# HakimNessah/th_rl

Hardware: AMD Instinct MI355X
Metric: env-steps/sec, 2-agent PD x 1M parallel games (higher is better)
Workload: dtype f32

## Files before the change

### th_rl_amd/csrc/thrl_wave_kernel.h

```cpp
#pragma once
#include <type_traits>
#include <utility>
#include "thrl_kernels.h"
#include "thrl_wave_lut.h"

#ifndef THRL_ABLATE
#define THRL_ABLATE 0
#endif

namespace thrl {

constexpr int kAblate = THRL_ABLATE;

typedef unsigned int v2u __attribute__((ext_vector_type(2)));

__device__ __forceinline__ v2u pack_halves(unsigned a, unsigned b) {
    return __builtin_amdgcn_permlane32_swap(a, b, false, false);
}

__device__ __forceinline__ unsigned lds_addr(const void* p) {
    return (unsigned)(uintptr_t)(__attribute__((address_space(3))) const void*)p;
}
template <typename QT>
__device__ __forceinline__ QT lds_load(unsigned addr) {
    typedef __attribute__((address_space(3))) QT lds_t;
    return *(const lds_t*)(uintptr_t)addr;
}
template <typename QT>
__device__ __forceinline__ void lds_store(unsigned addr, QT v) {
    typedef __attribute__((address_space(3))) QT lds_t;
    *(lds_t*)(uintptr_t)addr = v;
}

__device__ __forceinline__ void lds_inc(unsigned addr) {
    typedef unsigned __attribute__((may_alias)) u32_alias;
    typedef __attribute__((address_space(3))) u32_alias lds_u32;
    __hip_atomic_fetch_add((lds_u32*)(uintptr_t)addr, 1u, __ATOMIC_RELAXED, __HIP_MEMORY_SCOPE_WAVEFRONT);
}
__device__ __forceinline__ void lds_zero8(unsigned addr) {
    typedef unsigned long long __attribute__((may_alias)) u64_alias;
    typedef __attribute__((address_space(3))) u64_alias lds_u64;
    *(lds_u64*)(uintptr_t)addr = 0ull;
}

__device__ __forceinline__ unsigned bperm(unsigned byte_sel, unsigned v) {
    return (unsigned)__builtin_amdgcn_ds_bpermute((int)byte_sel, (int)v);
}

template <int CTRL>
__device__ __forceinline__ double dpp_mov64(double v) {
    const int lo = __double2loint(v), hi = __double2hiint(v);
    return __hiloint2double(__builtin_amdgcn_update_dpp(hi, hi, CTRL, 0xF, 0xF, false),
                            __builtin_amdgcn_update_dpp(lo, lo, CTRL, 0xF, 0xF, false));
}
template <int CTRL>
__device__ __forceinline__ uint32_t dpp_mov32(uint32_t v) {
    return (uint32_t)__builtin_amdgcn_update_dpp((int)v, (int)v, CTRL, 0xF, 0xF, false);
}

__device__ __forceinline__ float group8_allmax(float v) {
    asm("s_nop 1\n\t"
        "v_max_f32_dpp %0, %0, %0 quad_perm:[1,0,3,2] row_mask:0xf bank_mask:0xf\n\t"
        "s_nop 1\n\t"
        "v_max_f32_dpp %0, %0, %0 quad_perm:[2,3,0,1] row_mask:0xf bank_mask:0xf\n\t"
        "s_nop 1\n\t"
        "v_max_f32_dpp %0, %0, %0 row_half_mirror row_mask:0xf bank_mask:0xf"
        : "+v"(v));
    return v;
}
__device__ __forceinline__ double group8_allmax(double v) {
    v = fmax(v, dpp_mov64<0xB1>(v));
    v = fmax(v, dpp_mov64<0x4E>(v));
    v = fmax(v, dpp_mov64<0x141>(v));
    return v;
}
__device__ __forceinline__ void store_where(unsigned long long mask, unsigned addr, float v) {
    unsigned long long save;
    asm volatile("s_mov_b64 %0, exec\n\ts_mov_b64 exec, %1\n\tds_write_b32 %2, %3\n\ts_mov_b64 exec, %0"
                 : "=&s"(save) : "s"(mask), "v"(addr), "v"(v) : "memory");
}
__device__ __forceinline__ void store_where(unsigned long long mask, unsigned addr, double v) {
    unsigned long long save;
    asm volatile("s_mov_b64 %0, exec\n\ts_mov_b64 exec, %1\n\tds_write_b64 %2, %3\n\ts_mov_b64 exec, %0"
                 : "=&s"(save) : "s"(mask), "v"(addr), "v"(v) : "memory");
}
__device__ __forceinline__ void store_lanes(unsigned long long mask, long long* base, unsigned off, double v) {
    asm volatile("s_mov_b64 exec, %0\n\tglobal_store_dwordx2 %1, %2, %3\n\ts_mov_b64 exec, -1"
                 :: "s"(mask), "v"(off), "v"(v), "s"(base) : "memory");
}
template <int IMM>
__device__ __forceinline__ void store_key(unsigned key, unsigned want, unsigned addr, float v) {
    if constexpr (IMM >= 0)
        asm volatile("v_cmpx_eq_u32 vcc, %0, %1\n\tds_write_b32 %2, %3\n\ts_mov_b64 exec, -1"
                     :: "n"(IMM), "v"(key), "v"(addr), "v"(v) : "memory", "vcc");
    else
        asm volatile("v_cmpx_eq_u32 vcc, %0, %1\n\tds_write_b32 %2, %3\n\ts_mov_b64 exec, -1"
                     :: "s"(want), "v"(key), "v"(addr), "v"(v) : "memory", "vcc");
}
template <int IMM>
__device__ __forceinline__ void store_key(unsigned key, unsigned want, unsigned addr, double v) {
    if constexpr (IMM >= 0)
        asm volatile("v_cmpx_eq_u32 vcc, %0, %1\n\tds_write_b64 %2, %3\n\ts_mov_b64 exec, -1"
                     :: "n"(IMM), "v"(key), "v"(addr), "v"(v) : "memory", "vcc");
    else
        asm volatile("v_cmpx_eq_u32 vcc, %0, %1\n\tds_write_b64 %2, %3\n\ts_mov_b64 exec, -1"
                     :: "s"(want), "v"(key), "v"(addr), "v"(v) : "memory", "vcc");
}
constexpr unsigned kKeyShift = 25;
constexpr unsigned kKeyNone = 0x7Fu;
__device__ __forceinline__ float dpp_ror8(float v) { return __builtin_bit_cast(float, dpp_mov32<0x128>(__builtin_bit_cast(uint32_t, v))); }
__device__ __forceinline__ double dpp_ror8(double v) { return dpp_mov64<0x128>(v); }
__device__ __forceinline__ float max_of(float a, float b) { return fmaxf(a, b); }
__device__ __forceinline__ double max_of(double a, double b);
__device__ __forceinline__ float half32_allmax(float v) {
    v = group8_allmax(v);
    v = fmaxf(v, __builtin_bit_cast(float, dpp_mov32<0x140>(__builtin_bit_cast(uint32_t, v))));
    unsigned a = __builtin_bit_cast(unsigned, v), b = a;
    asm("" : "+v"(b));
    const v2u r = __builtin_amdgcn_permlane16_swap(a, b, false, false);
    const unsigned rx = r.x, ry = r.y;
// ... 380 lines not shown
template <int L>
__device__ __forceinline__ uint32_t writelane_imm(uint32_t old, uint32_t val) {
    asm("v_writelane_b32 %0, %1, %2" : "+v"(old) : "s"(val), "n"(L));
    return old;
}
template <int T0>
__device__ __forceinline__ void chain_group_affine(uint32_t& sq, uint32_t& sc, uint32_t Tq) {
    const uint32_t s1 = readlane_u(Tq, (int)sc) & 0xFFu;
    const uint32_t s2 = (readlane_u(Tq, (int)s1) >> 8) & 0xFFu;
    const uint32_t s3 = (readlane_u(Tq, (int)s2) >> 16) & 0xFFu;
    const uint32_t s4 = readlane_u(Tq, (int)s3) >> 24;
    const uint32_t w = pack16(sc, s2) | (pack16(s1, s3) << 8);
    sq = writelane_imm<T0>(sq, w);
    sc = s4;
}
__device__ __forceinline__ uint32_t play_affine(int seg, int n, int lane, uint32_t rw, uint32_t G0q, uint32_t G1q, unsigned mk_addr,
                                                int c, int m0, int m1, int& s) {
    const int s_entry = __builtin_amdgcn_readfirstlane(s);
    {
        const uint32_t kb = (uint32_t)c - ((rw & 1u) ? ((rw >> 8) & 0xFFu) * (uint32_t)m0 : 0u)
                                        - ((rw & 2u) ? ((rw >> 16) & 0xFFu) * (uint32_t)m1 : 0u);
        const unsigned ad = mk_addr + 16u * (unsigned)(lane >> 2) + (unsigned)(lane & 3);
        lds_store<unsigned char>(ad, (rw & 1u) ? (unsigned char)0 : (unsigned char)0xFF);
        lds_store<unsigned char>(ad + 4u, (rw & 2u) ? (unsigned char)0 : (unsigned char)0xFF);
        lds_store<unsigned char>(ad + 8u, (unsigned char)kb);
        __builtin_amdgcn_wave_barrier();
    }
    struct Q4 { v2u lo, hi; };
    auto loadq = [&](int g) {
        Q4 q;
        q.lo = lds_load<v2u>(mk_addr + 16u * (unsigned)g);
        q.hi = lds_load<v2u>(mk_addr + 16u * (unsigned)g + 8u);
        return q;
    };
    auto make = [&](const Q4& q) {
        asm volatile("" :: "v"(q.hi.y));
        return q.hi.x - (G0q & q.lo.x) - (G1q & q.lo.y);
    };
    uint32_t sq = 0u, sq_tail = 0u;
    uint32_t sc = (uint32_t)s_entry & 0xFFu;
    auto chain4 = [&](auto t0c, const int nn, const uint32_t Tq) {
        constexpr int t0 = decltype(t0c)::value;
        __builtin_amdgcn_sched_barrier(0);
        if (t0 + 4 <= nn) chain_group_affine<t0>(sq, sc, Tq);
        else {
#pragma unroll
            for (int j = 0; j < 4; j++) {
                if (t0 + j < nn) {
                    sq_tail = writelane_u(sq_tail, sc * 0x101u, t0 + j);
                    sc = (readlane_u(Tq, (int)sc) >> (8 * j)) & 0xFFu;
                }
            }
        }
        __builtin_amdgcn_sched_barrier(0);
    };
    Q4 qa = loadq(0), qb = loadq(1);
    uint32_t Ta = make(qa), Tb = 0u;
#define THRL_PLAYA2(G, N_)                                                                   \
    if ((G) * 4 < (N_)) {                                                                    \
        if ((G) * 4 + 8 < (N_)) qa = loadq((G) + 2 < 15 ? (G) + 2 : 15);                     \
        chain4(std::integral_constant<int, (G) * 4>(), (N_), Ta);                            \
        if ((G) * 4 + 4 < (N_)) {                                                            \
            Tb = make(qb);                                                                   \
            if ((G) * 4 + 12 < (N_)) qb = loadq((G) + 3 < 15 ? (G) + 3 : 15);                \
            chain4(std::integral_constant<int, (G) * 4 + 4>(), (N_), Tb);                    \
            if ((G) * 4 + 8 < (N_)) Ta = make(qa);                                           \
        }                                                                                    \
    }
#define THRL_PLAYA16(N_)                                                                     \
    THRL_PLAYA2(0, N_) THRL_PLAYA2(2, N_) THRL_PLAYA2(4, N_) THRL_PLAYA2(6, N_)              \
    THRL_PLAYA2(8, N_) THRL_PLAYA2(10, N_) THRL_PLAYA2(12, N_) THRL_PLAYA2(14, N_)
    if (n == 64) { THRL_PLAYA16(64) } else if (n == 36) { THRL_PLAYA16(36) } else { THRL_PLAYA16(n) }
#undef THRL_PLAYA16
#undef THRL_PLAYA2
    s = (int)(sc * 0x101u);
    uint32_t qd;
    asm("s_nop 1\n\tv_mov_b32_dpp %0, %1 quad_perm:[0,0,0,0] row_mask:0xf bank_mask:0xf" : "=v"(qd) : "v"(sq));
    const uint32_t un = ((qd >> (8u * (unsigned)(lane & 3))) & 0xFFu) * 0x101u;
    uint32_t out = lane < (n & ~3) ? un : sq_tail;
    if (seg == 0) out = writelane_imm<0>(out, (uint32_t)s_entry);
    return out;
}

template <typename QT, int NSEG, int NRSEG, bool NOISE, bool SWEEP, bool CYCLE, bool GREEDY = false, bool LOG = false, bool AFFINE = false>
__global__ void __launch_bounds__(1024)
__attribute__((amdgpu_waves_per_eu(sizeof(QT) == 8 ? 3 : (NOISE ? 4 : (NSEG <= 2 ? 5 : 4)))))
k_wave_episodes(const WaveArgs a) {
    extern __shared__ __attribute__((aligned(16))) unsigned char smem[];
    static_assert(!AFFINE || (sizeof(QT) == 4 && !NOISE && !SWEEP && !CYCLE && !GREEDY && NRSEG == 1 && kAblate == 0),
                  "closed-form play tables: plain float32 variants with one row register");
    constexpr bool kUnrollReplay = NSEG <= 2 && !(NOISE && sizeof(QT) == 8);
    const int lane = threadIdx.x & 63;
    const int wib = __builtin_amdgcn_readfirstlane((int)(threadIdx.x >> 6));
    const int A = a.A, W = a.win_rows, Tenv = a.T, epk = CYCLE ? a.epk : 1, T = a.T * epk, lo = a.row_lo;
    const int replay_from = CYCLE ? a.replay_from : 0;
    const WaveLut L = wave_lut_layout(A);

    {
        const uint32_t* src = reinterpret_cast<const uint32_t*>(a.lut_ns);
        uint32_t* dst = reinterpret_cast<uint32_t*>(smem);
        for (int k = threadIdx.x; k < (a.lut_bytes >> 2); k += blockDim.x) dst[k] = src[k];
    }
    __syncthreads();
    const unsigned lut_ns_lds = lds_addr(smem + L.ns_off);
    const double* lut_aq = reinterpret_cast<const double*>(smem + L.aq_off);
    const double* lut_sct = reinterpret_cast<const double*>(smem + L.sct_off);

    QT* tab0 = reinterpret_cast<QT*>(smem + a.lut_bytes + (size_t)wib * a.game_lds_bytes);
    QT* tab1 = tab0 + (W + 2) * A;
    const int half = lane >> 5;
    const unsigned tab0_off = lds_addr(tab0);
    const unsigned tab1_off = lds_addr(tab1);
    const int kk = (lane >> 3) & 3, jj = lane & 7;
    const unsigned perm_sel = (unsigned)((lane & 32) + 4 * jj + kk) << 2;
    const unsigned my_step = (unsigned)(4 * jj + kk);
    const unsigned row_shift = (unsigned)(7 * kk);
    const unsigned row_bytes = (unsigned)A * (unsigned)sizeof(QT);
    const int rdn = A < 3 ? 2 : (A <= 24 ? 3 : 4);
    const unsigned rd_base = (half ? tab1_off : tab0_off) + (unsigned)sizeof(QT) * (unsigned)min(rdn * jj, A - rdn);
    constexpr bool kLdsMK = sizeof(QT) == 4 && !NOISE && !GREEDY && NRSEG == 1 && !(kAblate & 6);
    const unsigned mk_addr = tab0_off + 2u * (unsigned)((W + 2) * A) * (unsigned)sizeof(QT);
    constexpr bool kArgmax21 = sizeof(QT) == 4;
    constexpr bool kMaskSched = !NOISE && !GREEDY;
    constexpr bool kParkLogs = !LOG && !CYCLE;

    const AgentParams& p0 = a.ag[0];
    const AgentParams& p1 = a.ag[1];
    const double inv_T_den = (double)Tenv;

    long long acc = 0, acc_hi = 0;
    const double log_scale = (lane & 2) ? a.log_scale[1] : a.log_scale[0];
    const int wave_gid = blockIdx.x * a.waves_per_block + wib;
    auto load_parked = [&](int pass) {
        return __hip_atomic_load(&a.partial[(size_t)wave_gid * 128 + 64 * pass + lane], __ATOMIC_RELAXED, __HIP_MEMORY_SCOPE_AGENT);
    };
    auto finish_parked = [&](long long p0w, long long p1w) {
#pragma unroll
        for (int pass = 0; pass < 2; pass++) {
            if (pass == 1 && a.n_episodes <= 16) break;
            double v = __longlong_as_double(pass ? p1w : p0w);
            if ((lane & 3) < 2) v = __ddiv_rn(v, inv_T_den);
            const long long vq = __double2ll_rn(__dmul_rn(v, log_scale));
            if (16 * pass + (lane >> 2) < a.n_episodes) { if (pass) acc_hi += vq; else acc += vq; }
        }
    };

    int g_claim = 0;
    if (lane == 0) g_claim = atomicAdd(a.next_game, 1);
    for (;;) {
        const int g = __builtin_amdgcn_readfirstlane(g_claim);
        if (g >= a.G) break;
        if (lane == 0) g_claim = atomicAdd(a.next_game, 1);
        const uint64_t gid = a.game_offset + (uint64_t)g;
        QT* __restrict__ q0 = reinterpret_cast<QT*>(a.q) + (int64_t)g * a.stride + p0.table_off;
        QT* __restrict__ q1 = reinterpret_cast<QT*>(a.q) + (int64_t)g * a.stride + p1.table_off;
        const double price0 = a.state[g];

        QT gamma_h = half ? HP<QT>::gamma(p1) : HP<QT>::gamma(p0);
        QT alpha_h = half ? HP<QT>::alpha(p1) : HP<QT>::alpha(p0);
        QT oma0 = HP<QT>::one_minus_alpha(p0), oma1 = HP<QT>::one_minus_alpha(p1);
        if (SWEEP && a.sw_gamma) gamma_h = HP<QT>::from_double(a.sw_gamma[(size_t)half * a.G + g]);
        if (SWEEP && a.sw_alpha) {
            alpha_h = HP<QT>::from_double(a.sw_alpha[(size_t)half * a.G + g]);
            oma0 = HP<QT>::from_double(__dsub_rn(1.0, a.sw_alpha[g]));
            oma1 = HP<QT>::from_double(__dsub_rn(1.0, a.sw_alpha[(size_t)a.G + g]));
        }
        double epsg0 = 0.0, epsg1 = 0.0;
        const bool sw_eps_on = SWEEP && a.sw_eps != nullptr;
        if (sw_eps_on) { epsg0 = a.sw_eps[g]; epsg1 = a.sw_eps[(size_t)a.G + g]; }
        const QT ag_h = HP<QT>::product(alpha_h, gamma_h);
        const double eend0 = (SWEEP && a.sw_eps_end) ? a.sw_eps_end[g] : p0.eps_end;
        const double eend1 = (SWEEP && a.sw_eps_end) ? a.sw_eps_end[(size_t)a.G + g] : p1.eps_end;
        const double estep0 = (SWEEP && a.sw_eps_step) ? a.sw_eps_step[g] : p0.eps_step;
        const double estep1 = (SWEEP && a.sw_eps_step) ? a.sw_eps_step[(size_t)a.G + g] : p1.eps_step;
        const double noise_prob_g = (SWEEP && a.sw_noise_prob) ? a.sw_noise_prob[g] : a.env.noise_prob;

        {
            const QT* s0 = q0 + lo * A;
            const QT* s1 = q1 + lo * A;
            const int n = W * A;
            for (int k0 = 0; k0 < n; k0 += 512) {
                QT v0[8], v1[8];
#pragma unroll
                for (int j = 0; j < 8; j++) {
                    const int k = min(k0 + j * 64 + lane, n - 1);
                    v0[j] = s0[k]; v1[j] = s1[k];
                }
#pragma unroll
                for (int j = 0; j < 8; j++) {
                    const int k = k0 + j * 64 + lane;
                    if (k < n) { tab0[k] = v0[j]; tab1[k] = v1[j]; }
                }
            }
        }
        int sp = __builtin_amdgcn_readfirstlane(encode32(price0, p0));
        int st = __builtin_amdgcn_readfirstlane(encode64(price0, p0));
        sp = min(max(sp, 0), a.rows - 1);
        st = min(max(st, 0), a.rows - 1);
        int spill0 = -1, spill1 = -1, sp_l, st_l;
        if (sp >= lo && sp < lo + W) sp_l = sp - lo; else { spill0 = sp; sp_l = W; }
        if (st == sp) st_l = sp_l;
        else if (st >= lo && st < lo + W) st_l = st - lo;
        else { spill1 = st; st_l = W + 1; }

        {
            if (spill0 >= 0 && lane < A) {
                tab0[W * A + lane] = q0[spill0 * A + lane];
                tab1[W * A + lane] = q1[spill0 * A + lane];
            }
            if (spill1 >= 0 && lane < A) {
                tab0[(W + 1) * A + lane] = q0[spill1 * A + lane];
                tab1[(W + 1) * A + lane] = q1[spill1 * A + lane];
            }
        }
        __builtin_amdgcn_wave_barrier();

        int s = sp_l | (st_l << 8);
        double last_price = price0;
        for (int e = 0; e < a.n_episodes; e += epk) {
            const uint32_t eg = (uint32_t)(a.first_episode + (uint64_t)e);

            uint32_t AM[NRSEG], R[NRSEG];
            uint32_t G0q = 0u, G1q = 0u;
#pragma unroll
            for (int k = 0; k < NRSEG; k++) {
                const int row = min(lane + 64 * k, W + 1);
                const QT* r0 = tab0 + row * A;
                const QT* r1 = tab1 + row * A;
                QT b0 = r0[0], b1 = r1[0];
                uint32_t i0 = 0, i1 = 0;
                if (kAblate & 16) {
                } else if (kArgmax21 && A == 21) {
                    i0 = argmax21_first(tab0_off + (unsigned)row * 84u);
                    i1 = argmax21_first(tab1_off + (unsigned)row * 84u);
                } else if (A == 21) {
#pragma unroll
                    for (int j = 1; j < 21; j++) {
                        const QT v0 = r0[j], v1 = r1[j];
                        if (v0 > b0) { b0 = v0; i0 = j; }
                        if (v1 > b1) { b1 = v1; i1 = j; }
                    }
                } else {
#pragma unroll 4
                    for (int j = 1; j < A; j++) {
                        const QT v0 = r0[j], v1 = r1[j];
                        if (v0 > b0) { b0 = v0; i0 = j; }
                        if (v1 > b1) { b1 = v1; i1 = j; }
                    }
                }
                if (kAblate & 16) { i0 = (uint32_t)(lane * 5) % (uint32_t)A; i1 = (uint32_t)(lane * 3) % (uint32_t)A; }
                AM[k] = i0 | (i1 << 8);
                R[k] = (i0 * (uint32_t)A * 2u) | (i1 << 17);
                if constexpr (AFFINE) {
                    G0q = i0 * ((uint32_t)a.aff_m0 * 0x01010101u);
                    G1q = i1 * ((uint32_t)a.aff_m1 * 0x01010101u);
                }
            }
            GreedyTables<GREEDY && NRSEG == 1> gt;
            gt.build(halves_sum(R[0]) + lut_ns_lds);

            uint32_t seq[NSEG], rwv[NSEG];
            unsigned explored_segs = 0u;
            double nav[NSEG];
#pragma unroll
            for (int seg = 0; seg < NSEG; seg++) {
                int n = min(64, T - seg * 64);
                asm volatile("" : "+s"(n));
                uint32_t rw;
                nav[seg] = 0.0;
                const int tcl = min(seg * 64 + lane, T - 1);
                const int ep = epk == 1 ? 0 : tcl / Tenv;
                const uint32_t st_in_ep = (uint32_t)(tcl - ep * Tenv);
                double eps0, eps1;
                if (sw_eps_on) { eps0 = epsg0; eps1 = epsg1; }
                else if (epk == 1) { eps0 = a.eps[e][0]; eps1 = a.eps[e][1]; }
                else { eps0 = a.eps[e + ep][0]; eps1 = a.eps[e + ep][1]; }
                if (a.inj_u) {
                    const int tt = tcl;
                    const size_t k = (((size_t)e * Tenv + tt) * 2) * (size_t)a.G + (size_t)g;
                    const uint32_t ex0 = a.inj_u[k] < eps0 ? 1u : 0u;
                    const uint32_t ex1 = a.inj_u[k + a.G] < eps1 ? 2u : 0u;
                    const uint32_t c0 = min((uint32_t)(uint8_t)a.inj_choice[k], (uint32_t)(A - 1));
                    const uint32_t c1 = min((uint32_t)(uint8_t)a.inj_choice[k + a.G], (uint32_t)(A - 1));
                    rw = ex0 | ex1 | (c0 << 8) | (c1 << 16);
                } else if (kAblate & 8) {
                    const uint32_t h = (uint32_t)(lane * 2654435761u) ^ eg;
                    rw = (h & 3u) | (((h >> 4) % (uint32_t)A) << 8) | (((h >> 12) % (uint32_t)A) << 16);
                } else {
                    uint32_t seed_lo = (uint32_t)a.seed, seed_hi = (uint32_t)(a.seed >> 32);
                    asm volatile("" : "+s"(seed_lo), "+s"(seed_hi));
                    const uint64_t seed_here = ((uint64_t)seed_hi << 32) | seed_lo;
                    const u32x4 x = draw_lanes(seed_here, gid, eg + (uint32_t)ep, st_in_ep, 0u);
                    const uint32_t ex0 = u01_32(x.x) < eps0 ? 1u : 0u;
                    const uint32_t ex1 = u01_32(x.z) < eps1 ? 2u : 0u;
                    rw = ex0 | ex1 | (__umulhi(x.y, (uint32_t)A) << 8) | (__umulhi(x.w, (uint32_t)A) << 16);
// ... 289 lines not shown
                    const uint32_t c1 = h1 & 1u;
                    const uint32_t c2 = ((h2 >> 1) & 1u) | ((c1 ^ 1u) & h2 & 1u);
                    const uint32_t c3 = ((h3 >> 2) & 1u) | ((c2 ^ 1u) & (((h3 >> 1) & 1u) | ((c1 ^ 1u) & h3 & 1u)));
                    bool quad_quiet = true;
                    if (NOISE) quad_quiet = ((__ballot((rwv[seg] & 4u) != 0u) >> (lane & 60)) & 0xFull) == 0ull;
                    const uint32_t same4 = ((quad_quiet && b0 == b1 && b1 == b2 && b2 == b3 && (b0 >> 24) == ((b0 >> 16) & 0xFFu)) ||
                                            (GREEDY && b0 == b2 && b1 == b3 && (b0 >> 24) == ((b1 >> 16) & 0xFFu) &&
                                             (b1 >> 24) == ((b0 >> 16) & 0xFFu) && (b0 >> 24) != (b1 >> 24))) ? 1u : 0u;
                    cutq = (c1 | (c2 << 1) | (c3 << 2)) & ((uint32_t)(pairs >> quad0) >> 1);
                    P = (b0 >> 24) | ((b1 >> 24) << 7) | ((b2 >> 24) << 14) | ((b3 >> 24) << 21) |
                        (cutq << 28) | (same4 << 31);
                    any_fixed = __ballot((P >> 31) != 0u) != 0ull;
                }

                const uint32_t pass_no = (uint32_t)__builtin_popcount(cutq & ((1u << ((uint32_t)lane & 3u)) - 1u));
                const uint32_t key_base = tab0_off + ((trains ? (quad0 & 28u) + pass_no : kKeyNone) << kKeyShift);
                const v2u woq = pack_halves(key_base + (cwv[seg] & 0xFFFFu) * kCellScale, key_base + (cwv[seg] >> 16) * kCellScale);

                bool seg_done = false;
                if (GREEDY && !(kAblate & 257) && !((explored_segs >> seg) & 1u)) {
                    const int nseg = min(64, T - seg * 64);
                    const uint32_t w = act[seg];
                    const uint32_t w1 = dpp_mov32<0x138>(w), w2 = dpp_mov32<0x138>(w1);
                    const uint32_t w3 = dpp_mov32<0x138>(w2), w4 = dpp_mov32<0x138>(w3);
                    const bool in_seg = lane < nseg;
                    const int period = __ballot(in_seg && lane >= 1 && w != w1) == 0ull ? 1
                                     : __ballot(in_seg && lane >= 2 && w != w2) == 0ull ? 2
                                     : __ballot(in_seg && lane >= 3 && w != w3) == 0ull ? 3
                                     : __ballot(in_seg && lane >= 4 && w != w4) == 0ull ? 4 : 0;
                    if (period > 0 && nseg >= period) {
                        uint32_t W[4];
#pragma unroll
                        for (int j = 0; j < 4; j++) W[j] = readlane_u(w, j);
                        bool ok = true;
#pragma unroll
                        for (int j = 0; j < 4; j++)
                            if (j < period) {
                                const uint32_t nxt_row = (W[(j + 1 < period) ? j + 1 : 0] >> 16) & 0xFFu;
                                ok = ok && (W[j] >> 24) == nxt_row;
#pragma unroll
                                for (int i = 0; i < j; i++) ok = ok && ((W[i] >> 16) & 0xFFu) != ((W[j] >> 16) & 0xFFu);
                            }
                        if (ok) {
                            seg_done = true;
                            const BlockOps<QT> ops0 = make_ops(snap[seg], 0, r0d, r1d, alpha_h);
                            const unsigned tabh = half ? tab1_off : tab0_off;
                            const unsigned wo_step = woq.x & ((1u << kKeyShift) - 1u);
                            if (period == 1) cyclic_segment<QT, 1>(ops0, wo_step, W, nseg, lane, tabh, A, row_bytes, ag_h, alpha_h, gamma_h);
                            else if (period == 2) cyclic_segment<QT, 2>(ops0, wo_step, W, nseg, lane, tabh, A, row_bytes, ag_h, alpha_h, gamma_h);
                            else if (period == 3) cyclic_segment<QT, 3>(ops0, wo_step, W, nseg, lane, tabh, A, row_bytes, ag_h, alpha_h, gamma_h);
                            else cyclic_segment<QT, 4>(ops0, wo_step, W, nseg, lane, tabh, A, row_bytes, ag_h, alpha_h, gamma_h);
                            __builtin_amdgcn_wave_barrier();
                        }
                    }
                }
#pragma unroll
                for (int k = 0; k < 2; k++) {
                    if (GREEDY && seg_done) break;
                    int nsub = __builtin_amdgcn_readfirstlane(min(32, T - seg * 64 - k * 32));
                    asm volatile("" : "+s"(nsub));
                    if (nsub <= 0) break;
                    BlockOps<QT> ops = make_ops(snap[seg], k, r0d, r1d, alpha_h);
                    ops.permute(perm_sel);
                    const unsigned wo = bperm(perm_sel, k ? woq.y : woq.x);
#define THRL_REPLAY(RDN_, FP_) replay_block<QT, RDN_, FP_, kUnrollReplay && RDN_ == 3, GREEDY>(P, k * 32, nsub, ops, wo, rd_base, row_shift, my_step, row_bytes, \
                                                          ag_h, alpha_h, gamma_h, half != 0, seg * 64 + k * 32, replay_from)
                    if (A > 24)      { if (any_fixed) THRL_REPLAY(4, true); else THRL_REPLAY(4, false); }
                    else if (A >= 3) { if (any_fixed) THRL_REPLAY(3, true); else THRL_REPLAY(3, false); }
                    else             { if (any_fixed) THRL_REPLAY(2, true); else THRL_REPLAY(2, false); }
#undef THRL_REPLAY
                }
            }

            if constexpr (kParkLogs) {
                const double v = (kAblate & 64) ? lr0 + lr1 + la0 + la1 : wave_sum4(lr0, lr1, la0, la1, lane);
                store_lanes(0xFull << (4 * (e & 3)), a.partial + ((size_t)wave_gid * kWaveMaxEpisodes + e) * 4, ((unsigned)lane & 3u) << 3, v);
            } else if (epk == 1) log_into(e, lr0, lr1, la0, la1, true);
            if (SWEEP) {
                epsg0 = __dadd_rn(eend0, __dmul_rn(__dsub_rn(epsg0, eend0), estep0));
                epsg1 = __dadd_rn(eend1, __dmul_rn(__dsub_rn(epsg1, eend1), estep1));
            }
        }

        {
            QT* d0 = q0 + lo * A;
            QT* d1 = q1 + lo * A;
            const int n = W * A;
            for (int k = lane; k < n; k += 64) { d0[k] = tab0[k]; d1[k] = tab1[k]; }
            if (spill0 >= 0 && lane < A) {
                q0[spill0 * A + lane] = tab0[W * A + lane];
                q1[spill0 * A + lane] = tab1[W * A + lane];
            }
            if (spill1 >= 0 && lane < A) {
                q0[spill1 * A + lane] = tab0[(W + 1) * A + lane];
                q1[spill1 * A + lane] = tab1[(W + 1) * A + lane];
            }
            if (lane == 0 && a.n_episodes > 0) a.state[g] = last_price;
            if (lane == 0 && sw_eps_on) { a.sw_eps[g] = epsg0; a.sw_eps[(size_t)a.G + g] = epsg1; }
        }
        __builtin_amdgcn_wave_barrier();

        const bool counting = a.counter && !(kAblate & 32);
        if constexpr (kParkLogs) {
            if (!counting && a.n_episodes > 0) {
                const long long p0w = load_parked(0), p1w = load_parked(1);
                finish_parked(p0w, p1w);
            }
        }
        if (counting) {
            const int cells = (W + 2) * A;
            typedef unsigned __attribute__((may_alias)) hist_u32;
            hist_u32* hist = reinterpret_cast<hist_u32*>(tab0);
            __builtin_amdgcn_fence(__ATOMIC_SEQ_CST, "wavefront");
            for (int k = lane; k < cells; k += 64) lds_zero8(tab0_off + 8u * (unsigned)k);
            __builtin_amdgcn_wave_barrier();
            const int n_cycles = a.n_episodes / epk;
            long long p0w = 0, p1w = 0;
            if constexpr (kParkLogs) { p0w = load_parked(0); p1w = load_parked(1); }
            for (int c0 = 0; c0 < n_cycles; c0 += 4) {
                unsigned w[4][NSEG];
#pragma unroll
                for (int j = 0; j < 4; j++)
#pragma unroll
                    for (int seg = 0; seg < NSEG; seg++)
                        w[j][seg] = __hip_atomic_load(
                            &a.tlog[(((size_t)wave_gid * kWaveMaxEpisodes + min(c0 + j, n_cycles - 1) * epk) * NSEG + seg) * 64 + lane],
                            __ATOMIC_RELAXED, __HIP_MEMORY_SCOPE_AGENT);
#pragma unroll
                for (int j = 0; j < 4; j++)
#pragma unroll
                    for (int seg = 0; seg < NSEG; seg++) {
                        const unsigned ww = w[j][seg];
                        if (c0 + j < n_cycles && ww != 0xFFFFFFFFu) {
                            lds_inc(tab0_off + (ww & 0xFFFFu));
                            lds_inc(tab0_off + (ww >> 16));
                        }
                    }
            }
            if constexpr (kParkLogs) finish_parked(p0w, p1w);
            __builtin_amdgcn_wave_barrier();
            int32_t* cw0 = a.counter + (int64_t)g * a.stride + p0.table_off;
            int32_t* cw1 = a.counter + (int64_t)g * a.stride + p1.table_off;
            const int nwin = W * A;
            auto add = [](int32_t* p, unsigned n) {
                if (n) __hip_atomic_fetch_add(p, (int32_t)n, __ATOMIC_RELAXED, __HIP_MEMORY_SCOPE_AGENT);
            };
            for (int k = lane; k < nwin; k += 64) {
                add(cw0 + lo * A + k, hist[k]);
                add(cw1 + lo * A + k, hist[cells + k]);
            }
            if (lane < 2 * A) {
                const int which = lane >= A, col = lane - which * A;
                const int grow_ = which ? spill1 : spill0;
                if (grow_ >= 0) {
                    add(cw0 + grow_ * A + col, hist[nwin + lane]);
                    add(cw1 + grow_ * A + col, hist[cells + nwin + lane]);
                }
            }
            __builtin_amdgcn_fence(__ATOMIC_SEQ_CST, "wavefront");
            __builtin_amdgcn_wave_barrier();
        }
    }
    a.partial[(size_t)wave_gid * 128 + lane] = acc;
    a.partial[(size_t)wave_gid * 128 + 64 + lane] = acc_hi;
}

template <typename QT, int NSEG, int NRSEG, bool NOISE, bool SWEEP, bool CYCLE, bool GREEDY, bool LOG, bool AFFINE = false>
static int launch_wave_t(const WaveArgs& a, int grid, int block, size_t lds, hipStream_t s) {
    auto kern = k_wave_episodes<QT, NSEG, NRSEG, NOISE, SWEEP, CYCLE, GREEDY, LOG, AFFINE>;
    if (lds > 64 * 1024) {
        const hipError_t e = hipFuncSetAttribute(reinterpret_cast<const void*>(kern),
                                                 hipFuncAttributeMaxDynamicSharedMemorySize, (int)lds);
        if (e != hipSuccess) return (int)e;
    }
    hipLaunchKernelGGL(kern, dim3(grid), dim3(block), lds, s, a);
    return (int)hipGetLastError();
}

template <typename QT, bool NOISE, bool SWEEP, bool CYCLE, bool GREEDY, bool LOG>
static int launch_wave_nl(const WaveArgs& a, int grid, int block, size_t lds, hipStream_t s) {
    const int nseg = (a.T * a.epk + 63) / 64;
    const int nrseg = (a.win_rows + 2 + 63) / 64;
    if (nrseg == 1) {
        switch (nseg) {
            case 1: return launch_wave_t<QT, 1, 1, NOISE, SWEEP, CYCLE, GREEDY, LOG>(a, grid, block, lds, s);
            case 2: return launch_wave_t<QT, 2, 1, NOISE, SWEEP, CYCLE, GREEDY, LOG>(a, grid, block, lds, s);
            case 3: return launch_wave_t<QT, 3, 1, NOISE, SWEEP, CYCLE, GREEDY, LOG>(a, grid, block, lds, s);
            case 4: return launch_wave_t<QT, 4, 1, NOISE, SWEEP, CYCLE, GREEDY, LOG>(a, grid, block, lds, s);
        }
    } else if (nrseg == 2) {
        switch (nseg) {
            case 1: return launch_wave_t<QT, 1, 2, NOISE, SWEEP, CYCLE, GREEDY, LOG>(a, grid, block, lds, s);
            case 2: return launch_wave_t<QT, 2, 2, NOISE, SWEEP, CYCLE, GREEDY, LOG>(a, grid, block, lds, s);
            case 3: return launch_wave_t<QT, 3, 2, NOISE, SWEEP, CYCLE, GREEDY, LOG>(a, grid, block, lds, s);
            case 4: return launch_wave_t<QT, 4, 2, NOISE, SWEEP, CYCLE, GREEDY, LOG>(a, grid, block, lds, s);
        }
    }
    return -1;
}

template <typename QT, bool NOISE, bool SWEEP, bool CYCLE, bool GREEDY = false>
static int launch_wave_n(const WaveArgs& a, int grid, int block, size_t lds, hipStream_t s) {
    if (a.game_reward_log || a.game_action_log) return launch_wave_nl<QT, NOISE, SWEEP, CYCLE, GREEDY, true>(a, grid, block, lds, s);
    return launch_wave_nl<QT, NOISE, SWEEP, CYCLE, GREEDY, false>(a, grid, block, lds, s);
}

}
```

Measured before the change: 48.65 billion.

## Batch and pipeline game-turnover memory traffic in the wave episode kernel

Result: no change. 48.92 billion, median of 6 (+0.6%).

```diff
diff --git a/profiles/turnover_chain.py b/profiles/turnover_chain.py
--- /dev/null
+++ b/profiles/turnover_chain.py
@@ -0,0 +1,188 @@
+#!/usr/bin/env python3
+import argparse
+import os
+import re
+import subprocess
+import sys
+import tempfile
+
+ROOT = os.path.dirname(os.path.dirname(os.path.abspath(__file__)))
+sys.path.insert(0, ROOT)
+
+HEADLINE = r"k_wave_episodesIfLi2ELi1ELb0ELb0ELb0ELb0ELb0ELb1E"
+
+
+def disassemble(csrc, src, defines):
+    from th_rl_amd.build import FLAGS
+    hipcc = os.environ.get("HIPCC", "/opt/rocm/bin/hipcc")
+    objdump = os.environ.get("LLVM_OBJDUMP", "/opt/rocm/llvm/bin/llvm-objdump")
+    flags = [f for f in FLAGS if f != "-shared"]
+    with tempfile.TemporaryDirectory() as tmp:
+        obj = os.path.join(tmp, "tu.o")
+        subprocess.check_call([hipcc] + flags + list(defines) + ["--cuda-device-only", "--no-gpu-bundle-output", "-c",
+                               os.path.join(csrc, src), "-o", obj], cwd=csrc)
+        return subprocess.check_output([objdump, "-d", "--no-show-raw-insn", obj], text=True)
+
+
+def symbols(listing):
+    out, cur, base = {}, None, 0
+    for line in listing.splitlines():
+        m = re.match(r"^([0-9a-f]+) <(\S+)>:", line)
+        if m:
+            cur, base = out.setdefault(m.group(2), []), int(m.group(1), 16)
+            continue
+        m = re.match(r"^\s+(\S+)\s*(.*?)\s*//\s*([0-9A-Fa-f]+):(.*)$", line)
+        if m and cur is not None:
+            t = re.search(r"<[^>]*\+0x[0-9a-f]+>", m.group(4))
+            cur.append((int(m.group(3), 16) - base, m.group(1), m.group(2) + (" " + t.group(0) if t else "")))
+    return out
+
+
+def loop_nest(ins):
+    index = {off: i for i, (off, _, _) in enumerate(ins)}
+    n = len(ins)
+    succ = [[] for _ in ins]
+    for i, (off, mn, ops) in enumerate(ins):
+        if mn.startswith("s_cbranch") or mn == "s_branch":
+            m = re.search(r"<[^>]*\+0x([0-9a-f]+)>", ops)
+            if m and int(m.group(1), 16) in index:
+                succ[i].append(index[int(m.group(1), 16)])
+        if mn == "s_setpc_b64":
+            for j in range(max(i - 4, 0), i):
+                m = re.match(r"(s\d+), \1, (0x[0-9a-f]+|-?\d+)$", ins[j + 1][2]) if ins[j][1] == "s_getpc_b64" and ins[j + 1][1] == "s_add_u32" else None
+                if m:
+                    d = int(m.group(2), 0)
+                    t = ins[j][0] + 4 + (d - (1 << 32) if d >= 1 << 31 else d)
+                    if t in index:
+                        succ[i].append(index[t])
+        if mn not in ("s_branch", "s_endpgm", "s_setpc_b64") and i + 1 < n:
+            succ[i].append(i + 1)
+    pred = [[] for _ in ins]
+    for i, ss in enumerate(succ):
+        for j in ss:
+            pred[j].append(i)
+
+    def components(nodes):
+        num, low, on, st, out, cnt = {}, {}, set(), [], [], 0
+        for root in nodes:
+            if root in num:
+                continue
+            work = [(root, 0)]
+            while work:
+                u, k = work.pop()
+                if k == 0:
+                    num[u] = low[u] = cnt
+                    cnt += 1
+                    st.append(u)
+                    on.add(u)
+                nxt = [v for v in succ[u] if v in nodes]
+                if k < len(nxt):
+                    work.append((u, k + 1))
+                    v = nxt[k]
+                    if v not in num:
+                        work.append((v, 0))
+                    elif v in on:
+                        low[u] = min(low[u], num[v])
+                    continue
+                if low[u] == num[u]:
+                    comp = set()
+                    while True:
+                        v = st.pop()
+                        on.discard(v)
+                        comp.add(v)
+                        if v == u:
+                            break
+                    if len(comp) > 1 or u in succ[u]:
+                        out.append(comp)
+                if work:
+                    low[work[-1][0]] = min(low[work[-1][0]], low[u])
+        return out
+
+    loops, todo = [], [(1, c) for c in components(set(range(n)))]
+    while todo:
+        level, comp = todo.pop()
+        loops.append((level, comp))
+        entries = {u for u in comp if any(q not in comp for q in pred[u])} or {min(comp)}
+        todo.extend((level + 1, c) for c in components(comp - entries))
+    return loops
+
+
+def classify(mn):
+    if mn == "s_waitcnt":
+        return "wait"
+    if mn.startswith("scratch_"):
+        return "scratch"
+    if mn.startswith(("global_", "flat_", "buffer_")):
+        return "vmem"
+    if mn.startswith("ds_"):
+        return "lds"
+    if mn.startswith(("s_load", "s_buffer_load")):
+        return "smem"
+    if mn.startswith("v_"):
+        return "valu"
+    if mn.startswith("s_"):
+        return "salu"
+    return "other"
+
+
+def chain_report(ins, quiet=False, out=sys.stdout):
+    loops = loop_nest(ins)
+    if not loops:
+        raise SystemExit("no loop in the symbol")
+    game = max((c for lv, c in loops if lv == 1), key=len)
+    epi = max((c for lv, c in loops if lv == 2 and c <= game), key=len)
+    eh = min(epi)
+    small = [c for lv, c in loops if lv >= 2 and c <= game and not c <= epi]
+    span = lambda body: (ins[min(body)][0], ins[max(body)][0])
+    print("game loop %d .. %d (%d instructions), episode loop %d .. %d (%d), symbol %d bytes" %
+          (span(game) + (len(game),) + span(epi) + (len(epi), ins[-1][0] + 4)), file=out)
+    turn = sorted(game - epi)
+    order = [i for i in turn if i > eh] + [i for i in turn if i < eh]
+    n_vm0 = n_wait_loop_vm = n_wait_loop_lgkm = n_scratch = n_vmem = n_lds = 0
+    prev = None
+    for i in order:
+        off, mn, ops = ins[i]
+        if prev is not None and i != prev + 1 and not quiet:
+            print("     --" + (" top of the game loop" if i < prev else ""), file=out)
+        prev = i
+        c = classify(mn)
+        if c not in ("wait", "scratch", "vmem", "lds", "smem"):
+            continue
+        depth = sum(1 for b in small if i in b)
+        if c == "wait":
+            n_vm0 += bool(re.search(r"vmcnt\(0\)", ops))
+            n_wait_loop_vm += bool(depth and "vmcnt" in ops)
+            n_wait_loop_lgkm += bool(depth and "lgkmcnt" in ops)
+        n_scratch += c == "scratch"
+        n_vmem += c == "vmem"
+        n_lds += c == "lds"
+        if not quiet:
+            print("%7d %s%-28s %s" % (off, "| " * depth, mn, ops), file=out)
+    print("turnover: %d instructions, vmem %d, lds %d, scratch %d, vmcnt(0) sites %d, waits inside loops: vmcnt %d, lgkmcnt %d" %
+          (len(turn), n_vmem, n_lds, n_scratch, n_vm0, n_wait_loop_vm, n_wait_loop_lgkm), file=out)
+    mix = {}
+    for i in epi:
+        mix[classify(ins[i][1])] = mix.get(classify(ins[i][1]), 0) + 1
+    print("episode loop: %d instructions: %s" % (len(epi), ", ".join("%s %d" % kv for kv in sorted(mix.items()))), file=out)
+    return {"game": span(game), "episode": span(epi), "vmcnt0": n_vm0, "loop_vm_waits": n_wait_loop_vm,
+            "loop_lgkm_waits": n_wait_loop_lgkm, "scratch": n_scratch, "episode_mix": mix}
+
+
+def main():
+    ap = argparse.ArgumentParser(description=__doc__.split("\n")[0])
+    ap.add_argument("--src", default="thrl_wave_f32a.hip")
+    ap.add_argument("--match", default=HEADLINE, help="regular expression that selects the kernel symbol")
+    ap.add_argument("--csrc", default=os.path.join(ROOT, "th_rl_amd", "csrc"))
+    ap.add_argument("--quiet", action="store_true", help="totals only")
+    ap.add_argument("--listing", help="read this llvm-objdump -d listing instead of compiling")
+    args, defines = ap.parse_known_args()
+    syms = symbols(open(args.listing).read() if args.listing else disassemble(args.csrc, args.src, defines))
+    names = [n for n in syms if re.search(args.match, n)]
+    if len(names) != 1:
+        raise SystemExit("--match selects %d symbols: %s" % (len(names), names or sorted(syms)))
+    print(names[0])
+    chain_report(syms[names[0]], args.quiet)
+
+
+if __name__ == "__main__":
+    main()
diff --git a/th_rl_amd/csrc/thrl_wave_kernel.h b/th_rl_amd/csrc/thrl_wave_kernel.h
--- a/th_rl_amd/csrc/thrl_wave_kernel.h
+++ b/th_rl_amd/csrc/thrl_wave_kernel.h
@@ -36,6 +36,11 @@
     typedef unsigned __attribute__((may_alias)) u32_alias;
     typedef __attribute__((address_space(3))) u32_alias lds_u32;
     __hip_atomic_fetch_add((lds_u32*)(uintptr_t)addr, 1u, __ATOMIC_RELAXED, __HIP_MEMORY_SCOPE_WAVEFRONT);
+}
+__device__ __forceinline__ unsigned lds_hist(unsigned addr) {
+    typedef unsigned __attribute__((may_alias)) u32_alias;
+    typedef __attribute__((address_space(3))) u32_alias lds_u32;
+    return *(const lds_u32*)(uintptr_t)addr;
 }
 __device__ __forceinline__ void lds_zero8(unsigned addr) {
     typedef unsigned long long __attribute__((may_alias)) u64_alias;
@@ -582,6 +587,18 @@
     return out;
 }
 
+#if defined(__HIP_DEVICE_COMPILE__)
+typedef const __attribute__((address_space(4))) WaveArgs* WaveArgsAgain;
+__device__ __forceinline__ WaveArgsAgain wave_args_again() {
+    WaveArgsAgain ka = (WaveArgsAgain)__builtin_amdgcn_kernarg_segment_ptr();
+    asm volatile("" : "+s"(ka));
+    return ka;
+}
+#else
+typedef const WaveArgs* WaveArgsAgain;
+__device__ __forceinline__ WaveArgsAgain wave_args_again() { return nullptr; }
+#endif
+
 template <typename QT, int NSEG, int NRSEG, bool NOISE, bool SWEEP, bool CYCLE, bool GREEDY = false, bool LOG = false, bool AFFINE = false>
 __global__ void __launch_bounds__(1024)
 __attribute__((amdgpu_waves_per_eu(sizeof(QT) == 8 ? 3 : (NOISE ? 4 : (NSEG <= 2 ? 5 : 4)))))
@@ -631,10 +648,8 @@
     long long acc = 0, acc_hi = 0;
     const double log_scale = (lane & 2) ? a.log_scale[1] : a.log_scale[0];
     const int wave_gid = blockIdx.x * a.waves_per_block + wib;
-    auto load_parked = [&](int pass) {
-        return __hip_atomic_load(&a.partial[(size_t)wave_gid * 128 + 64 * pass + lane], __ATOMIC_RELAXED, __HIP_MEMORY_SCOPE_AGENT);
-    };
     auto finish_parked = [&](long long p0w, long long p1w) {
+        asm volatile("" :: "v"(p1w));
 #pragma unroll
         for (int pass = 0; pass < 2; pass++) {
             if (pass == 1 && a.n_episodes <= 16) break;
@@ -645,16 +660,22 @@
         }
     };
 
-    int g_claim = 0;
-    if (lane == 0) g_claim = atomicAdd(a.next_game, 1);
-    for (;;) {
-        const int g = __builtin_amdgcn_readfirstlane(g_claim);
-        if (g >= a.G) break;
-        if (lane == 0) g_claim = atomicAdd(a.next_game, 1);
+    auto claim = [&]() {
+        int id = 0;
+        if (lane == 0) {
+            __attribute__((address_space(1))) int32_t* next = (__attribute__((address_space(1))) int32_t*)a.next_game;
+            asm volatile("" : "+v"(next));
+            id = __hip_atomic_fetch_add(next, 1, __ATOMIC_RELAXED, __HIP_MEMORY_SCOPE_AGENT);
+        }
+        return id;
+    };
+    int g = __builtin_amdgcn_readfirstlane(claim());
+    while (g < a.G) {
+        int g_claim = 0;
         const uint64_t gid = a.game_offset + (uint64_t)g;
         QT* __restrict__ q0 = reinterpret_cast<QT*>(a.q) + (int64_t)g * a.stride + p0.table_off;
         QT* __restrict__ q1 = reinterpret_cast<QT*>(a.q) + (int64_t)g * a.stride + p1.table_off;
-        const double price0 = a.state[g];
+        double price0 = 0.0;
 
         QT gamma_h = half ? HP<QT>::gamma(p1) : HP<QT>::gamma(p0);
         QT alpha_h = half ? HP<QT>::alpha(p1) : HP<QT>::alpha(p0);
@@ -675,24 +696,30 @@
         const double estep1 = (SWEEP && a.sw_eps_step) ? a.sw_eps_step[(size_t)a.G + g] : p1.eps_step;
         const double noise_prob_g = (SWEEP && a.sw_noise_prob) ? a.sw_noise_prob[g] : a.env.noise_prob;
 
+        int lane_p = lane;
+        asm volatile("" : "+v"(lane_p));
         {
             const QT* s0 = q0 + lo * A;
             const QT* s1 = q1 + lo * A;
             const int n = W * A;
-            for (int k0 = 0; k0 < n; k0 += 512) {
-                QT v0[8], v1[8];
-#pragma unroll
-                for (int j = 0; j < 8; j++) {
-                    const int k = min(k0 + j * 64 + lane, n - 1);
+            constexpr int kInBatch = sizeof(QT) == 4 ? 14 : 8;
+            for (int k0 = 0; k0 < n; k0 += 64 * kInBatch) {
+                QT v0[kInBatch], v1[kInBatch];
+#pragma unroll
+                for (int j = 0; j < kInBatch; j++) {
+                    const int k = min(k0 + j * 64 + lane_p, n - 1);
                     v0[j] = s0[k]; v1[j] = s1[k];
                 }
-#pragma unroll
-                for (int j = 0; j < 8; j++) {
-                    const int k = k0 + j * 64 + lane;
-                    if (k < n) { tab0[k] = v0[j]; tab1[k] = v1[j]; }
-                }
-            }
-        }
+                if (k0 == 0) { price0 = a.state[g]; g_claim = claim(); }
+#pragma unroll
+                for (int j = 0; j < kInBatch; j++) {
+                    const unsigned k = (unsigned)min(k0 + j * 64 + lane_p, n - 1);
+                    lds_store<QT>(tab0_off + (unsigned)sizeof(QT) * k, v0[j]);
+                    lds_store<QT>(tab1_off + (unsigned)sizeof(QT) * k, v1[j]);
+                }
+            }
+        }
+        const int g_next = __builtin_amdgcn_readfirstlane(g_claim);
         int sp = __builtin_amdgcn_readfirstlane(encode32(price0, p0));
         int st = __builtin_amdgcn_readfirstlane(encode64(price0, p0));
         sp = min(max(sp, 0), a.rows - 1);
@@ -704,13 +731,13 @@
         else { spill1 = st; st_l = W + 1; }
 
         {
-            if (spill0 >= 0 && lane < A) {
-                tab0[W * A + lane] = q0[spill0 * A + lane];
-                tab1[W * A + lane] = q1[spill0 * A + lane];
-            }
-            if (spill1 >= 0 && lane < A) {
-                tab0[(W + 1) * A + lane] = q0[spill1 * A + lane];
-                tab1[(W + 1) * A + lane] = q1[spill1 * A + lane];
+            if (spill0 >= 0 && lane_p < A) {
+                tab0[W * A + lane_p] = q0[spill0 * A + lane_p];
+                tab1[W * A + lane_p] = q1[spill0 * A + lane_p];
+            }
+            if (spill1 >= 0 && lane_p < A) {
+                tab0[(W + 1) * A + lane_p] = q0[spill1 * A + lane_p];
+                tab1[(W + 1) * A + lane_p] = q1[spill1 * A + lane_p];
             }
         }
         __builtin_amdgcn_wave_barrier();
@@ -1166,84 +1193,135 @@
             }
         }
 
+        int lane_t = lane;
+        asm volatile("" : "+v"(lane_t));
+        const WaveArgsAgain ka = wave_args_again();
+        const int64_t goff = (int64_t)g * ka->stride;
+        const int A_t = ka->A, W_t = ka->win_rows, lo_t = ka->row_lo, n_episodes_t = ka->n_episodes;
+        const unsigned tab0_t = lds_addr(smem + ka->lut_bytes + (size_t)wib * ka->game_lds_bytes);
+        const unsigned tab1_t = tab0_t + (unsigned)((W_t + 2) * A_t) * (unsigned)sizeof(QT);
+        constexpr int kTurnBatch = 4;
+
         {
-            QT* d0 = q0 + lo * A;
-            QT* d1 = q1 + lo * A;
-            const int n = W * A;
-            for (int k = lane; k < n; k += 64) { d0[k] = tab0[k]; d1[k] = tab1[k]; }
-            if (spill0 >= 0 && lane < A) {
-                q0[spill0 * A + lane] = tab0[W * A + lane];
-                q1[spill0 * A + lane] = tab1[W * A + lane];
-            }
-            if (spill1 >= 0 && lane < A) {
-                q0[spill1 * A + lane] = tab0[(W + 1) * A + lane];
-                q1[spill1 * A + lane] = tab1[(W + 1) * A + lane];
-            }
-            if (lane == 0 && a.n_episodes > 0) a.state[g] = last_price;
-            if (lane == 0 && sw_eps_on) { a.sw_eps[g] = epsg0; a.sw_eps[(size_t)a.G + g] = epsg1; }
+            QT* qg0 = reinterpret_cast<QT*>(ka->q) + goff + ka->ag[0].table_off;
+            QT* qg1 = reinterpret_cast<QT*>(ka->q) + goff + ka->ag[1].table_off;
+            QT* d0 = qg0 + lo_t * A_t;
+            QT* d1 = qg1 + lo_t * A_t;
+            const int n = W_t * A_t;
+            for (int k0 = 0; k0 < n; k0 += 64 * kTurnBatch) {
+                QT v0[kTurnBatch], v1[kTurnBatch];
+#pragma unroll
+                for (int j = 0; j < kTurnBatch; j++) {
+                    const unsigned k = (unsigned)min(k0 + j * 64 + lane_t, n - 1);
+                    v0[j] = lds_load<QT>(tab0_t + (unsigned)sizeof(QT) * k);
+                    v1[j] = lds_load<QT>(tab1_t + (unsigned)sizeof(QT) * k);
+                }
+#pragma unroll
+                for (int j = 0; j < kTurnBatch; j++) {
+                    const int k = min(k0 + j * 64 + lane_t, n - 1);
+                    d0[k] = v0[j]; d1[k] = v1[j];
+                }
+            }
+            if (spill0 >= 0 && lane_t < A_t) {
+                qg0[spill0 * A_t + lane_t] = lds_load<QT>(tab0_t + (unsigned)sizeof(QT) * (unsigned)(W_t * A_t + lane_t));
+                qg1[spill0 * A_t + lane_t] = lds_load<QT>(tab1_t + (unsigned)sizeof(QT) * (unsigned)(W_t * A_t + lane_t));
+            }
+            if (spill1 >= 0 && lane_t < A_t) {
+                qg0[spill1 * A_t + lane_t] = lds_load<QT>(tab0_t + (unsigned)sizeof(QT) * (unsigned)((W_t + 1) * A_t + lane_t));
+                qg1[spill1 * A_t + lane_t] = lds_load<QT>(tab1_t + (unsigned)sizeof(QT) * (unsigned)((W_t + 1) * A_t + lane_t));
+            }
+            if (lane_t == 0 && n_episodes_t > 0) ka->state[g] = last_price;
+            if (lane_t == 0 && sw_eps_on) { a.sw_eps[g] = epsg0; a.sw_eps[(size_t)a.G + g] = epsg1; }
         }
         __builtin_amdgcn_wave_barrier();
 
-        const bool counting = a.counter && !(kAblate & 32);
+        const bool counting = ka->counter && !(kAblate & 32);
+        auto load_parked = [&](int pass) {
+            return __hip_atomic_load(&ka->partial[(size_t)wave_gid * 128 + 64 * pass + lane_t], __ATOMIC_RELAXED, __HIP_MEMORY_SCOPE_AGENT);
+        };
         if constexpr (kParkLogs) {
-            if (!counting && a.n_episodes > 0) {
+            if (!counting && n_episodes_t > 0) {
                 const long long p0w = load_parked(0), p1w = load_parked(1);
                 finish_parked(p0w, p1w);
             }
         }
         if (counting) {
-            const int cells = (W + 2) * A;
-            typedef unsigned __attribute__((may_alias)) hist_u32;
-            hist_u32* hist = reinterpret_cast<hist_u32*>(tab0);
+            const int cells = (W_t + 2) * A_t;
             __builtin_amdgcn_fence(__ATOMIC_SEQ_CST, "wavefront");
-            for (int k = lane; k < cells; k += 64) lds_zero8(tab0_off + 8u * (unsigned)k);
-            __builtin_amdgcn_wave_barrier();
-            const int n_cycles = a.n_episodes / epk;
-            long long p0w = 0, p1w = 0;
-            if constexpr (kParkLogs) { p0w = load_parked(0); p1w = load_parked(1); }
-            for (int c0 = 0; c0 < n_cycles; c0 += 4) {
-                unsigned w[4][NSEG];
-#pragma unroll
-                for (int j = 0; j < 4; j++)
+            constexpr int kLogBatch = NSEG <= 2 ? 8 / NSEG : 2;
+            const int epk_t = CYCLE ? ka->epk : 1;
+            const int n_cycles = n_episodes_t / epk_t;
+            const int last_cycle = max(n_cycles, 1) - 1;
+            const uint32_t* tl = ka->tlog + (size_t)wave_gid * kWaveMaxEpisodes * NSEG * 64 + lane_t;
+            auto issue = [&](unsigned (&w)[kLogBatch][NSEG], int c0) {
+#pragma unroll
+                for (int j = 0; j < kLogBatch; j++)
 #pragma unroll
                     for (int seg = 0; seg < NSEG; seg++)
-                        w[j][seg] = __hip_atomic_load(
-                            &a.tlog[(((size_t)wave_gid * kWaveMaxEpisodes + min(c0 + j, n_cycles - 1) * epk) * NSEG + seg) * 64 + lane],
-                            __ATOMIC_RELAXED, __HIP_MEMORY_SCOPE_AGENT);
-#pragma unroll
-                for (int j = 0; j < 4; j++)
+                        w[j][seg] = __hip_atomic_load(tl + ((size_t)(min(c0 + j, last_cycle) * epk_t) * NSEG + seg) * 64,
+                                                      __ATOMIC_RELAXED, __HIP_MEMORY_SCOPE_AGENT);
+            };
+            auto consume = [&](const unsigned (&w)[kLogBatch][NSEG], int c0) {
+#pragma unroll
+                for (int j = 0; j < kLogBatch; j++)
 #pragma unroll
                     for (int seg = 0; seg < NSEG; seg++) {
                         const unsigned ww = w[j][seg];
                         if (c0 + j < n_cycles && ww != 0xFFFFFFFFu) {
-                            lds_inc(tab0_off + (ww & 0xFFFFu));
-                            lds_inc(tab0_off + (ww >> 16));
+                            lds_inc(tab0_t + (ww & 0xFFFFu));
+                            lds_inc(tab0_t + (ww >> 16));
                         }
                     }
+            };
+            long long p0w = 0, p1w = 0;
+            if constexpr (kParkLogs) { p0w = load_parked(0); p1w = load_parked(1); }
+            unsigned wa[kLogBatch][NSEG], wb[kLogBatch][NSEG];
+            issue(wa, 0);
+            for (int k = lane_t; k < cells; k += 64) lds_zero8(tab0_t + 8u * (unsigned)k);
+            __builtin_amdgcn_wave_barrier();
+            for (int c0 = 0;;) {
+                issue(wb, c0 + kLogBatch);
+                consume(wa, c0);
+                c0 += 2 * kLogBatch;
+                if (c0 >= n_cycles) { consume(wb, c0 - kLogBatch); break; }
+                issue(wa, c0);
+                consume(wb, c0 - kLogBatch);
             }
             if constexpr (kParkLogs) finish_parked(p0w, p1w);
             __builtin_amdgcn_wave_barrier();
-            int32_t* cw0 = a.counter + (int64_t)g * a.stride + p0.table_off;
-            int32_t* cw1 = a.counter + (int64_t)g * a.stride + p1.table_off;
-            const int nwin = W * A;
+            int32_t* cw0 = ka->counter + goff + ka->ag[0].table_off;
+            int32_t* cw1 = ka->counter + goff + ka->ag[1].table_off;
+            const int nwin = W_t * A_t;
             auto add = [](int32_t* p, unsigned n) {
                 if (n) __hip_atomic_fetch_add(p, (int32_t)n, __ATOMIC_RELAXED, __HIP_MEMORY_SCOPE_AGENT);
             };
-            for (int k = lane; k < nwin; k += 64) {
-                add(cw0 + lo * A + k, hist[k]);
-                add(cw1 + lo * A + k, hist[cells + k]);
-            }
-            if (lane < 2 * A) {
-                const int which = lane >= A, col = lane - which * A;
+            for (int k0 = 0; k0 < nwin; k0 += 64 * kTurnBatch) {
+                unsigned h0[kTurnBatch], h1[kTurnBatch];
+#pragma unroll
+                for (int j = 0; j < kTurnBatch; j++) {
+                    const unsigned k = (unsigned)min(k0 + j * 64 + lane_t, nwin - 1);
+                    h0[j] = lds_hist(tab0_t + 4u * k);
+                    h1[j] = lds_hist(tab0_t + 4u * ((unsigned)cells + k));
+                }
+#pragma unroll
+                for (int j = 0; j < kTurnBatch; j++) {
+                    const int k = k0 + j * 64 + lane_t;
+                    add(cw0 + lo_t * A_t + k, k < nwin ? h0[j] : 0u);
+                    add(cw1 + lo_t * A_t + k, k < nwin ? h1[j] : 0u);
+                }
+            }
+            if (lane_t < 2 * A_t) {
+                const int which = lane_t >= A_t, col = lane_t - which * A_t;
                 const int grow_ = which ? spill1 : spill0;
                 if (grow_ >= 0) {
-                    add(cw0 + grow_ * A + col, hist[nwin + lane]);
-                    add(cw1 + grow_ * A + col, hist[cells + nwin + lane]);
+                    add(cw0 + grow_ * A_t + col, lds_hist(tab0_t + 4u * (unsigned)(nwin + lane_t)));
+                    add(cw1 + grow_ * A_t + col, lds_hist(tab0_t + 4u * (unsigned)(cells + nwin + lane_t)));
                 }
             }
             __builtin_amdgcn_fence(__ATOMIC_SEQ_CST, "wavefront");
             __builtin_amdgcn_wave_barrier();
         }
+        g = g_next;
     }
     a.partial[(size_t)wave_gid * 128 + lane] = acc;
     a.partial[(size_t)wave_gid * 128 + 64 + lane] = acc_hi;
```
